# siboehm/NormalizingFlowNetwork

Hardware: AMD Instinct MI355X
Metric: log_prob evals/sec (whole node), 10-flow planar+radial chain, y_dim=1 (higher is better)
Workload: dtype f32; 1 GPU; C2: y_dim=1, (planar,radial)x5 chain, batch 2^24 per GPU; batch_per_gpu=16777216, global_batch=16777216, y_dim=1, param_width=32, trainable_base=True, math=fast, parallelism=dp1, mode=forward

## Files before the change

### normalizingflownetwork_amd/csrc/nfn_bf16.h

```cpp
#pragma once
#include <hip/hip_runtime.h>
#include <stdint.h>

namespace nfn {

typedef float f32x4v __attribute__((ext_vector_type(4)));
typedef unsigned int u32x4v __attribute__((ext_vector_type(4)));
typedef __bf16 bf16x2v __attribute__((ext_vector_type(2)));
typedef __bf16 bf16x8v __attribute__((ext_vector_type(8)));
typedef short s16x4v __attribute__((ext_vector_type(4)));
typedef __attribute__((address_space(3))) s16x4v lds_s16x4v;

__device__ __forceinline__ uint32_t pk_bf16(float a, float b) {
  const bf16x2v v = {(__bf16)a, (__bf16)b};
  return __builtin_bit_cast(uint32_t, v);
}
__device__ __forceinline__ float bf16_lo(uint32_t u) { return __uint_as_float(u << 16); }
__device__ __forceinline__ float bf16_hi(uint32_t u) { return __uint_as_float(u & 0xffff0000u); }
__device__ __forceinline__ void split3_pk(float a, float b, uint32_t& hi, uint32_t& mi, uint32_t& lo) {
  hi = pk_bf16(a, b);
  const float ra = a - bf16_lo(hi), rb = b - bf16_hi(hi);
  mi = pk_bf16(ra, rb);
  lo = pk_bf16(ra - bf16_lo(mi), rb - bf16_hi(mi));
}
__device__ __forceinline__ bf16x8v frag8(uint32_t a, uint32_t b, uint32_t c, uint32_t d) {
  const u32x4v v = {a, b, c, d};
  return __builtin_bit_cast(bf16x8v, v);
}
__device__ __forceinline__ bf16x8v frag8(u32x4v v) { return __builtin_bit_cast(bf16x8v, v); }
__device__ __forceinline__ f32x4v mfma_bf16(bf16x8v a, bf16x8v b, f32x4v c) {
  return __builtin_amdgcn_mfma_f32_16x16x32_bf16(a, b, c, 0, 0, 0);
}

}
```

### normalizingflownetwork_amd/csrc/nfn_dense.hip

```cpp
#include "nfn_bf16.h"
#include "nfn_launch.h"

namespace nfn {
namespace {

typedef float f32x4v __attribute__((ext_vector_type(4)));

template <int DM, bool FAST, int NVH>
__global__ void __launch_bounds__(kMaxBlock) chain_dense_kernel(DenseArgs da) {
  const ChainArgs& a = da.c;
  extern __shared__ float lds[];
  __shared__ double red[2 * kMaxBlock / 64];
  const int tid = threadIdx.x;
  const int lane = tid & 63;
  const int wid = tid >> 6;
  const int H = da.H;
  const int QH = H >> 2;
  const int SH = da.h_lds_stride;
  const int S = a.lds_stride;
  const int P = a.P;
  const int NN = (P + 15) >> 4;
  const int NK = QH;
  const int NP = NN * 16;
  float* wl = lds;
// ... 133 lines not shown
  const int ak = lane >> 4;
  constexpr bool kBReg = QH * NN <= 16;
  float bvr[kBReg ? QH : 1][kBReg ? NN : 1];
  if constexpr (kBReg && !SB) {
#pragma unroll
    for (int ks = 0; ks < QH; ++ks)
#pragma unroll
      for (int nt = 0; nt < NN; ++nt) bvr[ks][nt] = wl[(4 * ks + ak) * NP + 16 * nt + am];
  }
  bf16x8v wsb[SB ? NN : 1][3];
  if constexpr (SB) {
#pragma unroll
    for (int nt = 0; nt < NN; ++nt) {
      uint32_t w1[4], w2[4], w3[4];
#pragma unroll
      for (int q = 0; q < 4; ++q) {
        const int k0 = 8 * (ak & 1) + 2 * q;
        split3_pk(wl[k0 * NP + 16 * nt + am], wl[(k0 + 1) * NP + 16 * nt + am], w1[q], w2[q], w3[q]);
      }
      const bool lo = ak < 2;
      wsb[nt][0] = lo ? frag8(w1[0], w1[1], w1[2], w1[3]) : frag8(w2[0], w2[1], w2[2], w2[3]);
      wsb[nt][1] = lo ? frag8(w3[0], w3[1], w3[2], w3[3]) : frag8(w2[0], w2[1], w2[2], w2[3]);
      wsb[nt][2] = frag8(w1[0], w1[1], w1[2], w1[3]);
    }
  }
  const int64_t hs = da.h_rowstride;
  const int64_t ntiles = a.ntiles;
  const int64_t u0 = (int64_t)blockIdx.x * (blockDim.x >> 6) + wid;
  const int64_t ustep = (int64_t)gridDim.x * (blockDim.x >> 6);
  const bool norm = a.y_mean != nullptr;
  float ymean = 0.0f, ystd = 1.0f, corr = 0.0f;
  if (norm) {
    ymean = a.y_mean[0];
    ystd = a.y_std[0];
    corr = f_log<true>(ystd);
  }
  const int yoff = lane * (int)a.y_bstride * 4;
  const int hoff = (r0 * (int)hs + 4 * c4) * 4;
  const int kstep = RSTEP * (int)hs * 4;
  float4 buf[QH];
  float ybuf;
  auto issue = [&](int64_t tile) {
    if (diag_ablate_loads(a)) tile = u0;
    const int64_t b0 = tile * 64;
    const int64_t nr = max((int64_t)0, min((int64_t)64, a.B - b0));
    const int64_t b0c = nr > 0 ? b0 : 0;
    const auto ry = tile_rsrc(a.y + b0c * a.y_bstride, nr > 0 ? ((nr - 1) * a.y_bstride + 1) * 4 : 0);
    ybuf = __builtin_bit_cast(float, __builtin_amdgcn_raw_buffer_load_b32(ry, yoff, 0, 0));
    const auto rh = tile_rsrc(da.h + b0c * hs, nr > 0 ? ((nr - 1) * hs + H) * 4 : 0);
#pragma unroll
    for (int k = 0; k < QH; ++k)
      buf[k] = __builtin_bit_cast(float4, __builtin_amdgcn_raw_buffer_load_b128(rh, hoff, k * kstep, kNT));
  };
  double acc_sum = 0.0;
  int nfc = 0;
  __amdgpu_buffer_rsrc_t pend_r = tile_rsrc(a.out, 0);
  float pend_v = 0.0f;
  auto flush = [&]() {
    __builtin_amdgcn_raw_buffer_store_b32(__builtin_bit_cast(uint32_t, pend_v), pend_r, lane * 4, 0, kNT);
  };
  issue(u0);
  flush();
  for (int64_t tile = u0; tile < ntiles; tile += ustep) {
    const int64_t b0 = tile * 64;
    const int64_t nr = max((int64_t)0, min((int64_t)64, a.B - b0));
    if constexpr (SB) {
#pragma unroll
      for (int k = 0; k < QH; ++k) {
        uint32_t p1[2], p2[2], p3[2];
        split3_pk(buf[k].x, buf[k].y, p1[0], p2[0], p3[0]);
        split3_pk(buf[k].z, buf[k].w, p1[1], p2[1], p3[1]);
        uint32_t* dst = reinterpret_cast<uint32_t*>(hl) + (r0 + k * RSTEP) * 8 + 2 * c4;
        *reinterpret_cast<uint2*>(dst) = make_uint2(p1[0], p1[1]);
        *reinterpret_cast<uint2*>(dst + kSbPlane) = make_uint2(p2[0], p2[1]);
        *reinterpret_cast<uint2*>(dst + 2 * kSbPlane) = make_uint2(p3[0], p3[1]);
      }
    } else {
#pragma unroll
      for (int k = 0; k < QH; ++k) {
        float* dst = hl + l0 + k * RSTEP * SH;
        dst[0] = buf[k].x;
        dst[1] = buf[k].y;
        dst[2] = buf[k].z;
        dst[3] = buf[k].w;
      }
    }
    const float z0 = norm ? f_div<true>(ybuf - ymean, ystd) : ybuf;
    wave_lds_sync();
    issue(tile + ustep);
    flush();
    if constexpr (SB) {
      const uint32_t* pl = reinterpret_cast<const uint32_t*>(hl) + 4 * (ak & 1);
      const int pa = ak < 2 ? 2 * kSbPlane : kSbPlane, pc = ak < 2 ? kSbPlane : 0;
      f32x4v acc[NN][4];
#pragma unroll
      for (int mt = 0; mt < 4; ++mt) {
        const uint32_t* row = pl + (16 * mt + am) * 8;
        const bf16x8v h0 = frag8(*reinterpret_cast<const u32x4v*>(row + pa));
        const bf16x8v h1 = frag8(*reinterpret_cast<const u32x4v*>(row));
        const bf16x8v h2 = frag8(*reinterpret_cast<const u32x4v*>(row + pc));
#pragma unroll
        for (int nt = 0; nt < NN; ++nt) {
          acc[nt][mt] = mfma_bf16(h0, wsb[nt][0], f32x4v{0.0f, 0.0f, 0.0f, 0.0f});
          acc[nt][mt] = mfma_bf16(h1, wsb[nt][1], acc[nt][mt]);
          acc[nt][mt] = mfma_bf16(h2, wsb[nt][2], acc[nt][mt]);
        }
      }
#pragma unroll
      for (int nt = 0; nt < NN; ++nt) {
        const int n = 16 * nt + am;
        if (n < P) {
          const float bn = da.bias ? da.bias[n] : 0.0f;
#pragma unroll
          for (int mt = 0; mt < 4; ++mt)
            *reinterpret_cast<f32x4v*>(tl + n * kCS + 16 * mt + 4 * ak) = acc[nt][mt] + bn;
        }
      }
    } else {
    float av[4][QH];
#pragma unroll
    for (int mt = 0; mt < 4; ++mt)
#pragma unroll
      for (int ks = 0; ks < QH; ++ks) av[mt][ks] = hl[(16 * mt + am) * SH + 4 * ks + ak];
#pragma unroll
    for (int nt = 0; nt < NN; ++nt) {
      f32x4v acc[4];
#pragma unroll
      for (int mt = 0; mt < 4; ++mt) acc[mt] = f32x4v{0.0f, 0.0f, 0.0f, 0.0f};
#pragma unroll
      for (int ks = 0; ks < QH; ++ks) {
        const float bv = kBReg ? bvr[kBReg ? ks : 0][kBReg ? nt : 0] : wl[(4 * ks + ak) * NP + 16 * nt + am];
#pragma unroll
        for (int mt = 0; mt < 4; ++mt) acc[mt] = __builtin_amdgcn_mfma_f32_16x16x4f32(av[mt][ks], bv, acc[mt], 0, 0, 0);
      }
      const int n = 16 * nt + am;
      if (n < P) {
        const float bn = da.bias ? da.bias[n] : 0.0f;
#pragma unroll
        for (int mt = 0; mt < 4; ++mt)
          *reinterpret_cast<f32x4v*>(tl + n * kCS + 16 * mt + 4 * ak) = acc[mt] + bn;
      }
    }
    }
    wave_lds_sync();
    const float lp = (a.prog.K <= 16 ? eval_chain1_fast<true, kCS, CM, false>(z0, tl + lane, a)
                                     : eval_chain1_fast<false, kCS, kChainLoop, false>(z0, tl + lane, a)) - corr;
    if (lane < nr) {
      acc_sum += (double)lp;
      nfc += nonfinite1(lp);
    }
    pend_v = lp;
    pend_r = tile_rsrc(a.out && nr > 0 ? a.out + b0 : a.out, a.out ? nr * 4 : 0);
    wave_lds_sync();
  }
  flush();
  if (a.partials) {
    write_partial(a.partials, acc_sum, nfc, red, a.out_sum, a.epoch, a.pair_base);
  }
}

template <int QH, int NN, int CM = kChainLoop>
__global__ void __launch_bounds__(kMaxBlock) posterior_dense1_kernel(DenseArgs da) {
  const ChainArgs& a = da.c;
  extern __shared__ float lds[];
  __shared__ double red[2 * kMaxBlock / 64];
  constexpr int RSTEP = 64 / QH;
  constexpr int kNT = 2;
  const int tid = threadIdx.x;
  const int lane = tid & 63;
  const int wid = __builtin_amdgcn_readfirstlane(tid >> 6);
  const int SH = da.h_lds_stride;
  const int P = a.P;
  const int S = a.S;
  float* hl = lds + wid * dense1_wave_floats(P, SH);
  float* tl = hl;
  const int r0 = lane / QH, c4 = lane % QH;
  const int l0 = r0 * SH + 4 * c4;
  const int am = lane & 15, ak = lane >> 4;
  const int64_t hs = da.h_rowstride;
  const int64_t ntiles = a.ntiles;
  const int64_t u0 = (int64_t)blockIdx.x * (blockDim.x >> 6) + wid;
  const int64_t ustep = (int64_t)gridDim.x * (blockDim.x >> 6);
  const bool norm = a.y_mean != nullptr;
  float ymean = 0.0f, ystd = 1.0f, corr = 0.0f;
  if (norm) {
    ymean = a.y_mean[0];
    ystd = a.y_std[0];
    corr = f_log<true>(ystd);
  }
  const int yoff = lane * (int)a.y_bstride * 4;
  const int hoff = (r0 * (int)hs + 4 * c4) * 4;
  const int kstep = RSTEP * (int)hs * 4;
  int woff[QH][NN];
  bool wcol[NN];
#pragma unroll
  for (int nt = 0; nt < NN; ++nt) {
    wcol[nt] = 16 * nt + am < P;
#pragma unroll
    for (int ks = 0; ks < QH; ++ks) woff[ks][nt] = wcol[nt] ? ((4 * ks + ak) * P + 16 * nt + am) * 4 : 0;
  }
  float4 buf[QH];
  float ybuf;
  float wbuf[QH][NN], bbuf[NN];
  auto issue = [&](int64_t tile, int sd) {
    const int64_t b0 = tile * 64;
    const int64_t nr = max((int64_t)0, min((int64_t)64, a.B - b0));
    const int64_t b0c = nr > 0 ? b0 : 0;
    const auto ry = tile_rsrc(a.y + b0c * a.y_bstride, nr > 0 ? ((nr - 1) * a.y_bstride + 1) * 4 : 0);
    ybuf = __builtin_bit_cast(float, __builtin_amdgcn_raw_buffer_load_b32(ry, yoff, 0, 0));
    const auto rh = tile_rsrc(da.h + sd * da.h_drawstride + b0c * hs, nr > 0 ? ((nr - 1) * hs + 4 * QH) * 4 : 0);
#pragma unroll
    for (int k = 0; k < QH; ++k)
      buf[k] = __builtin_bit_cast(float4, __builtin_amdgcn_raw_buffer_load_b128(rh, hoff, k * kstep, kNT));
    const auto rw = tile_rsrc(da.W + sd * da.w_drawstride, nr > 0 ? (int64_t)4 * QH * P * 4 : 0);
#pragma unroll
    for (int ks = 0; ks < QH; ++ks)
#pragma unroll
      for (int nt = 0; nt < NN; ++nt)
        wbuf[ks][nt] = __builtin_bit_cast(float, __builtin_amdgcn_raw_buffer_load_b32(rw, woff[ks][nt], 0, 0));
    const auto rb = tile_rsrc(da.bias ? da.bias + sd * da.b_drawstride : da.W, (da.bias && nr > 0) ? P * 4 : 0);
#pragma unroll
    for (int nt = 0; nt < NN; ++nt)
      bbuf[nt] = __builtin_bit_cast(float, __builtin_amdgcn_raw_buffer_load_b32(rb, (16 * nt + am) * 4, 0, 0));
  };
  double acc_sum = 0.0;
  int nfc = 0;
  __amdgpu_buffer_rsrc_t pend_r = tile_rsrc(a.out, 0);
  float pend_v = 0.0f;
  auto flush = [&]() {
    __builtin_amdgcn_raw_buffer_store_b32(__builtin_bit_cast(uint32_t, pend_v), pend_r, lane * 4, 0, kNT);
  };
  issue(u0, 0);
  flush();
  for (int64_t tile = u0; tile < ntiles; tile += ustep) {
    const int64_t b0 = tile * 64;
    const int64_t nr = max((int64_t)0, min((int64_t)64, a.B - b0));
    float m = -INFINITY, lacc = 0.0f;
    for (int sd = 0; sd < S; ++sd) {
#pragma unroll
      for (int k = 0; k < QH; ++k) {
        float* dst = hl + l0 + k * RSTEP * SH;
        dst[0] = buf[k].x;
        dst[1] = buf[k].y;
        dst[2] = buf[k].z;
        dst[3] = buf[k].w;
      }
      float wv[QH][NN], bv[NN];
#pragma unroll
      for (int nt = 0; nt < NN; ++nt) {
        bv[nt] = bbuf[nt];
#pragma unroll
        for (int ks = 0; ks < QH; ++ks) wv[ks][nt] = wcol[nt] ? wbuf[ks][nt] : 0.0f;
      }
      const float z0 = norm ? f_div<true>(ybuf - ymean, ystd) : ybuf;
      wave_lds_sync();
      const bool last = sd + 1 == S;
      issue(last ? tile + ustep : tile, last ? 0 : sd + 1);
      flush();
      pend_r = tile_rsrc(a.out, 0);
      float av[4][QH];
#pragma unroll
      for (int mt = 0; mt < 4; ++mt)
#pragma unroll
        for (int ks = 0; ks < QH; ++ks) av[mt][ks] = hl[(16 * mt + am) * SH + 4 * ks + ak];
#pragma unroll
      for (int nt = 0; nt < NN; ++nt) {
        f32x4v acc[4];
#pragma unroll
        for (int mt = 0; mt < 4; ++mt) acc[mt] = f32x4v{0.0f, 0.0f, 0.0f, 0.0f};
#pragma unroll
        for (int ks = 0; ks < QH; ++ks)
#pragma unroll
          for (int mt = 0; mt < 4; ++mt) acc[mt] = __builtin_amdgcn_mfma_f32_16x16x4f32(av[mt][ks], wv[ks][nt], acc[mt], 0, 0, 0);
        const int n = 16 * nt + am;
        if (n < P) {
#pragma unroll
          for (int mt = 0; mt < 4; ++mt)
            *reinterpret_cast<f32x4v*>(tl + n * kCS + 16 * mt + 4 * ak) = acc[mt] + bv[nt];
        }
      }
      wave_lds_sync();
      const float lp = (a.prog.K <= 16 ? eval_chain1_fast<true, kCS, CM, false>(z0, tl + lane, a)
                                       : eval_chain1_fast<false, kCS, kChainLoop, false>(z0, tl + lane, a)) - corr;
      lse_push<true>(m, lacc, lp);
      wave_lds_sync();
    }
    const float res = lse_finish<true>(m, lacc, S);
    if (lane < nr) {
      acc_sum += (double)res;
      nfc += nonfinite1(res);
    }
    pend_v = res;
    pend_r = tile_rsrc(a.out && nr > 0 ? a.out + b0 : a.out, a.out ? nr * 4 : 0);
  }
  flush();
  if (a.partials) {
    write_partial(a.partials, acc_sum, nfc, red, a.out_sum, a.epoch, a.pair_base);
  }
}

template <int DM, bool FAST>
__global__ void __launch_bounds__(kMaxBlock) posterior_dense_kernel(DenseArgs da) {
  const ChainArgs& a = da.c;
  extern __shared__ float lds[];
  __shared__ double red[2 * kMaxBlock / 64];
  const int tid = threadIdx.x;
// ... 203 lines not shown
        for (int ks = 0; ks < QH; ++ks) av[mt][ks] = hl[(16 * mt + am) * SH + 4 * ks + ak];
#pragma unroll
      for (int nt = 0; nt < NNMAX; ++nt) {
        if (nt < NN) {
          f32x4v acc[4];
#pragma unroll
          for (int mt = 0; mt < 4; ++mt) acc[mt] = f32x4v{0.0f, 0.0f, 0.0f, 0.0f};
#pragma unroll
          for (int ks = 0; ks < QH; ++ks)
#pragma unroll
            for (int mt = 0; mt < 4; ++mt)
              acc[mt] = __builtin_amdgcn_mfma_f32_16x16x4f32(av[mt][ks], wv[ks][nt], acc[mt], 0, 0, 0);
          const int n = 16 * nt + am;
          if (n < P) {
#pragma unroll
            for (int mt = 0; mt < 4; ++mt) {
#pragma unroll
              for (int i = 0; i < 4; ++i) tl[(16 * mt + 4 * ak + i) * S + n] = acc[mt][i] + bv[nt];
            }
          }
        }
      }
      wave_lds_sync();
      float z[DM];
#pragma unroll
      for (int j = 0; j < DM; ++j) z[j] = z0[j];
      const float lp = eval_chain<DM, true>(z, tl + lane * S, a) - corr;
      lse_push<true>(m, lacc, lp);
      wave_lds_sync();
    }
    const float res = lse_finish<true>(m, lacc, ND);
    if (lane < nr) {
      acc_sum += (double)res;
      nfc += nonfinite1(res);
    }
    pend_v = res;
    pend_r = tile_rsrc(a.out && nr > 0 ? a.out + b0 : a.out, a.out ? nr * 4 : 0);
  }
  flush();
  if (a.partials) {
    write_partial(a.partials, acc_sum, nfc, red, a.out_sum, a.epoch, a.pair_base);
  }
}

template <int DM, int QH>
void launch_pdp(const DenseArgs& da, hipStream_t s, int64_t* grid_out) {
  auto kfn = posterior_densep_kernel<DM, QH>;
  const size_t lds = (size_t)(4 * (64 * da.h_lds_stride + 64 * da.c.lds_stride) + 16) * sizeof(float);
  const int64_t grid = persistent_grid(kfn, kMaxBlock, lds, (da.c.ntiles + 3) / 4);
  *grid_out = std::max<int64_t>(1, grid);
  nfn_launch(kfn, dim3((unsigned)*grid_out), dim3(kMaxBlock), lds, s, da);
}

template <int DM>
bool launch_pdp_h(const DenseArgs& da, hipStream_t s, int64_t* g) {
  switch (da.H >> 2) {
    case 1: launch_pdp<DM, 1>(da, s, g); return true;
    case 2: launch_pdp<DM, 2>(da, s, g); return true;
    case 4: launch_pdp<DM, 4>(da, s, g); return true;
  }
  return false;
}

template <int QH, int CM>
void launch_pd1_form(const DenseArgs& da, hipStream_t s, int64_t* grid_out) {
  const int nn = (da.c.P + 15) >> 4;
  const size_t lds = (size_t)(4 * dense1_wave_floats(da.c.P, da.h_lds_stride) + 16) * sizeof(float);
  auto kfn = nn <= 1 ? posterior_dense1_kernel<QH, 1, CM>
                     : (nn == 2 ? posterior_dense1_kernel<QH, 2, CM> : (nn == 3 ? posterior_dense1_kernel<QH, 3, CM>
                                                                                : posterior_dense1_kernel<QH, 4, CM>));
  int64_t grid = persistent_grid(kfn, kMaxBlock, lds, (da.c.ntiles + 3) / 4);
  *grid_out = std::max<int64_t>(1, grid);
  nfn_launch(kfn, dim3((unsigned)*grid_out), dim3(kMaxBlock), lds, s, da);
}

#ifndef NFN_DENSE_HP
template <int QH>
void launch_pd1(const DenseArgs& da, hipStream_t s, int64_t* grid_out) {
  int cm = env_int("NFN_CHAIN_FORM", -1);
  if (cm < 0 && hpair_types(da.c) >= 0) cm = kChainHPair;
  if (cm == kChainHPair && launch_dense1_hpair(hpair_types(da.c), true, da, s, grid_out)) return;
  if (cm == kChainLoop)
    launch_pd1_form<QH, kChainLoop>(da, s, grid_out);
  else
    launch_pd1_form<QH, kChainPairs>(da, s, grid_out);
}

template <int DM, bool FAST>
void launch_pd(const DenseArgs& da, hipStream_t s, int64_t* grid_out) {
  auto kfn = posterior_dense_kernel<DM, FAST>;
  const size_t lds = (size_t)(4 * (64 * da.h_lds_stride + 64 * da.c.lds_stride) + 16) * sizeof(float);
  const int64_t grid = persistent_grid(kfn, kMaxBlock, lds, (da.c.ntiles + 3) / 4);
  *grid_out = std::max<int64_t>(1, grid);
  nfn_launch(kfn, dim3((unsigned)*grid_out), dim3(kMaxBlock), lds, s, da);
}

template <bool FAST>
bool launch_pd_dm(int dm, const DenseArgs& da, hipStream_t s, int64_t* g) {
  const ChainArgs& a = da.c;
  if constexpr (FAST) {
    if (dm == 1 && a.d == 1 && env_int("NFN_DENSE1", 1) != 0 && da.h_rowstride * 256 < ((int64_t)1 << 31) &&
        a.y_bstride * 256 < ((int64_t)1 << 31)) {
      switch (da.H >> 2) {
        case 1: launch_pd1<1>(da, s, g); return true;
        case 2: launch_pd1<2>(da, s, g); return true;
        case 4: launch_pd1<4>(da, s, g); return true;
        case 8: launch_pd1<8>(da, s, g); return true;
      }
    }
  }
  if constexpr (FAST) {
    if (dm >= 2 && a.d >= 2 && da.H <= 16 && env_int("NFN_DENSEP", 1) != 0 && da.h_rowstride * 256 < ((int64_t)1 << 31) &&
        a.y_bstride * 256 < ((int64_t)1 << 31)) {
      bool ok = false;
      switch (dm) {
        case 2: ok = launch_pdp_h<2>(da, s, g); break;
        case 4: ok = launch_pdp_h<4>(da, s, g); break;
        case 8: ok = launch_pdp_h<8>(da, s, g); break;
      }
      if (ok) return true;
    }
  }
  switch (dm) {
    case 1: launch_pd<1, FAST>(da, s, g); return true;
    case 2: launch_pd<2, FAST>(da, s, g); return true;
    case 4: launch_pd<4, FAST>(da, s, g); return true;
    case 8: launch_pd<8, FAST>(da, s, g); return true;
  }
  return false;
}

#endif

constexpr int kDenseSplitBf16 = 1;
template <int QH, int CM>
void launch_d1_form(const DenseArgs& da, hipStream_t s, int64_t* grid_out) {
  const int nn = (da.c.P + 15) >> 4;
  bool sb = false;
  if constexpr (QH == 4) sb = nn <= 2 && env_int("NFN_DENSE_SB", kDenseSplitBf16) != 0;
  const int wf = sb ? dense1_sb_wave_floats(da.c.P, da.h_lds_stride) : dense1_wave_floats(da.c.P, da.h_lds_stride);
  const size_t lds = (size_t)(4 * QH * nn * 16 + 4 * wf + 16) * sizeof(float);
  auto kfn = nn <= 1 ? chain_dense1_kernel<QH, 1, CM>
                     : (nn == 2 ? chain_dense1_kernel<QH, 2, CM> : (nn == 3 ? chain_dense1_kernel<QH, 3, CM>
                                                                           : chain_dense1_kernel<QH, 4, CM>));
  if constexpr (QH == 4) {
    if (sb) kfn = nn <= 1 ? chain_dense1_kernel<QH, 1, CM, true> : chain_dense1_kernel<QH, 2, CM, true>;
  }
  int64_t grid = persistent_grid(kfn, kMaxBlock, lds, (da.c.ntiles + 3) / 4);
  *grid_out = std::max<int64_t>(1, grid);
  nfn_launch(kfn, dim3((unsigned)*grid_out), dim3(kMaxBlock), lds, s, da);
}

#ifndef NFN_DENSE_HP
template <int QH>
void launch_d1(const DenseArgs& da, size_t , hipStream_t s, int64_t* grid_out) {
  int cm = env_int("NFN_CHAIN_FORM", -1);
  if (cm < 0 && hpair_types(da.c) >= 0) cm = kChainHPair;
  if (cm == kChainHPair && launch_dense1_hpair(hpair_types(da.c), false, da, s, grid_out)) return;
#ifdef NFN_DIAG
  if (cm == kStaticProg && (da.c.P + 15) >> 4 == 2 && da.c.prog.K == kStaticK[0] &&
      da.c.prog.types[0] == kStaticTypes[0]) {
    launch_d1_form<QH, kStaticProg>(da, s, grid_out);
    return;
  }
  if (cm == kChainLoop) {
    launch_d1_form<QH, kChainLoop>(da, s, grid_out);
    return;
  }
#endif
  launch_d1_form<QH, kChainPairs>(da, s, grid_out);
}
#endif

#ifndef NFN_DENSE_HP
template <int DM, bool FAST, int NVH>
void launch_d(const DenseArgs& da, size_t lds, hipStream_t s, int64_t* grid_out) {
  auto kfn = chain_dense_kernel<DM, FAST, NVH>;
  const int64_t grid = persistent_grid(kfn, kMaxBlock, lds, (da.c.ntiles + 3) / 4);
  *grid_out = std::max<int64_t>(1, grid);
  nfn_launch(kfn, dim3((unsigned)*grid_out), dim3(kMaxBlock), lds, s, da);
}

template <int DM, bool FAST>
bool launch_d_h(int nvh, const DenseArgs& da, size_t lds, hipStream_t s, int64_t* g) {
  switch (nvh) {
    case 1: launch_d<DM, FAST, 1>(da, lds, s, g); return true;
    case 2: launch_d<DM, FAST, 2>(da, lds, s, g); return true;
    case 4: launch_d<DM, FAST, 4>(da, lds, s, g); return true;
    case 8: launch_d<DM, FAST, 8>(da, lds, s, g); return true;
    case 16: launch_d<DM, FAST, 16>(da, lds, s, g); return true;
  }
  return false;
}

template <bool FAST>
bool launch_d_dm(int dm, int nvh, const DenseArgs& da, size_t lds, hipStream_t s, int64_t* g) {
  const ChainArgs& a = da.c;
  if constexpr (FAST) {
    if (dm == 1 && a.d == 1 && env_int("NFN_DENSE1", 1) != 0 && da.h_rowstride * 256 < ((int64_t)1 << 31) &&
        a.y_bstride * 256 < ((int64_t)1 << 31)) {
      switch (nvh) {
        case 1: launch_d1<1>(da, lds, s, g); return true;
        case 2: launch_d1<2>(da, lds, s, g); return true;
        case 4: launch_d1<4>(da, lds, s, g); return true;
        case 8: launch_d1<8>(da, lds, s, g); return true;
      }
    }
  }
  switch (dm) {
    case 1: return launch_d_h<1, FAST>(nvh, da, lds, s, g);
    case 2: return launch_d_h<2, FAST>(nvh, da, lds, s, g);
    case 4: return launch_d_h<4, FAST>(nvh, da, lds, s, g);
    case 8: return launch_d_h<8, FAST>(nvh, da, lds, s, g);
  }
  return false;
}

#endif

}

#ifdef NFN_DENSE_HP
#define NFN_CAT2(a, b) a##b
#define NFN_CAT(a, b) NFN_CAT2(a, b)
#define NFN_DENSE_HP_FN NFN_CAT(launch_dense1_hpair_, NFN_DENSE_HP)
bool NFN_DENSE_HP_FN(bool post, const DenseArgs& da, hipStream_t s, int64_t* g) {
  constexpr int CM = hpair_form(NFN_DENSE_HP / 3, NFN_DENSE_HP % 3, 1);
  switch (da.H >> 2) {
    case 1: post ? launch_pd1_form<1, CM>(da, s, g) : launch_d1_form<1, CM>(da, s, g); return true;
    case 2: post ? launch_pd1_form<2, CM>(da, s, g) : launch_d1_form<2, CM>(da, s, g); return true;
    case 4: post ? launch_pd1_form<4, CM>(da, s, g) : launch_d1_form<4, CM>(da, s, g); return true;
    case 8: post ? launch_pd1_form<8, CM>(da, s, g) : launch_d1_form<8, CM>(da, s, g); return true;
  }
  return false;
}
#else
bool launch_dense1_hpair(int sel, bool post, const DenseArgs& da, hipStream_t s, int64_t* grid) {
  switch (sel) {
    case 0: return launch_dense1_hpair_0(post, da, s, grid);
    case 1: return launch_dense1_hpair_1(post, da, s, grid);
    case 3: return launch_dense1_hpair_3(post, da, s, grid);
    case 4: return launch_dense1_hpair_4(post, da, s, grid);
  }
  return false;
}

bool launch_dense(bool fast, int dm, int nvh, const DenseArgs& da, size_t lds, hipStream_t s, int64_t* grid) {
  return fast ? launch_d_dm<true>(dm, nvh, da, lds, s, grid) : launch_d_dm<false>(dm, nvh, da, lds, s, grid);
}

bool launch_posterior_dense(bool fast, int dm, const DenseArgs& da, hipStream_t s, int64_t* grid) {
  return fast ? launch_pd_dm<true>(dm, da, s, grid) : launch_pd_dm<false>(dm, da, s, grid);
}
#endif

}
```

### normalizingflownetwork_amd/csrc/nfn_device.h

```cpp
#pragma once

#include <hip/hip_runtime.h>

#include <math.h>
#include <stdint.h>
#include <stdlib.h>
#include <string.h>

#include <algorithm>

#include "nfn.h"

#pragma clang fp contract(on)

#if defined(__HIP_DEVICE_COMPILE__) && !defined(__gfx950__)
#error "the nfn kernels are written for gfx950 (MI355X) only"
#endif

namespace nfn {

constexpr int kMaxBlock = 256;
constexpr int kLdsTileBudget = 48 * 1024;
constexpr int kLdsMaxBytes = 156 * 1024;
constexpr float kSoftplusThr = 13.942384719848633f;
// ... 486 lines not shown
}

#define NFN_PAIR_SWITCH(sel, CALL) \
  switch (sel) {                   \
    case 0: CALL(0, 0); break;     \
    case 1: CALL(0, 1); break;     \
    case 2: CALL(0, 2); break;     \
    case 3: CALL(1, 0); break;     \
    case 4: CALL(1, 1); break;     \
    case 5: CALL(1, 2); break;     \
    case 6: CALL(2, 0); break;     \
    case 7: CALL(2, 1); break;     \
    default: CALL(2, 2); break;    \
  }

__device__ __forceinline__ int type1(uint32_t types, int k) { return (int)((types >> ((2 * k) & 31)) & 3u); }

template <int ST = 1, bool ACCM = true>
__device__ __forceinline__ float chain1_fast_pairs(float& z, const float* row, uint32_t types, int K, int P) {
  float l2 = 0.0f;
  int ia = type1(types, 0), ib = type1(types, 1);
  int offa = max(P - size1(ia), 0), offb = max(offa - size1(ib), 0);
  float pa[3], pb[3];
  read3c<ST>(pa, row, offa);
  read3c<ST>(pb, row, offb);
#pragma unroll 1
  for (int k = 0; k + 1 < K; k += 2) {
    const int ian = type1(types, k + 2), ibn = type1(types, k + 3);
    const int offan = max(offb - size1(ian), 0), offbn = max(offan - size1(ibn), 0);
    float pna[3], pnb[3];
    read3c<ST>(pna, row, offan);
    read3c<ST>(pnb, row, offbn);
#define NFN_FWD(A, B) flow_pair1<A, B, ACCM>(z, l2, pa, pb)
    NFN_PAIR_SWITCH(ia * 3 + ib, NFN_FWD)
#undef NFN_FWD
    ia = ian;
    ib = ibn;
    offb = offbn;
#pragma unroll
    for (int i = 0; i < 3; ++i) {
      pa[i] = pna[i];
      pb[i] = pnb[i];
    }
  }
  if (K & 1) l2 += __builtin_amdgcn_logf(fabsf(flow1_fast<ACCM>(ia, z, pa)));
  return l2;
}

template <int IA, int IB, int U, int ST = 1, bool ACCM = true>
__device__ __forceinline__ float chain1_fast_hpairs(float& z, const float* row, int K, int P) {
  constexpr int SA = IA == NFN_FLOW_AFFINE ? 2 : 3, SB = IB == NFN_FLOW_AFFINE ? 2 : 3, SP = SA + SB;
  float l2 = 0.0f;
  int off = P;
  const int np = K >> 1;
  int p = 0;
  if constexpr (U == 0) {
    float pa[3], pb[3];
    read3c<ST>(pa, row, max(off - SA, 0));
    read3c<ST>(pb, row, max(off - SP, 0));
#pragma unroll 1
    for (; p < np; ++p) {
      off -= SP;
      float pna[3], pnb[3];
      read3c<ST>(pna, row, max(off - SA, 0));
      read3c<ST>(pnb, row, max(off - SP, 0));
      flow_pair1<IA, IB, ACCM>(z, l2, pa, pb);
#pragma unroll
      for (int i = 0; i < 3; ++i) {
        pa[i] = pna[i];
        pb[i] = pnb[i];
      }
    }
    if (K & 1) l2 += __builtin_amdgcn_logf(fabsf(flow1_fast<ACCM>(IA, z, pa)));
    return l2;
  }
#pragma unroll 1
  for (; p + U <= np; p += U) {
    float pa[U > 0 ? U : 1][3], pb[U > 0 ? U : 1][3];
#pragma unroll
    for (int u = 0; u < U; ++u) {
      read3c<ST>(pa[u], row, off - u * SP - SA);
      read3c<ST>(pb[u], row, off - u * SP - SP);
    }
#pragma unroll
    for (int u = 0; u < U; ++u) flow_pair1<IA, IB, ACCM>(z, l2, pa[u], pb[u]);
    off -= U * SP;
  }
#pragma unroll 1
  for (; p < np; ++p) {
    float pa[3], pb[3];
    read3c<ST>(pa, row, off - SA);
    read3c<ST>(pb, row, off - SP);
    flow_pair1<IA, IB, ACCM>(z, l2, pa, pb);
    off -= SP;
  }
  if (K & 1) {
    float pa[3];
    read3c<ST>(pa, row, off - SA);
    l2 += __builtin_amdgcn_logf(fabsf(flow1_fast<ACCM>(IA, z, pa)));
  }
  return l2;
}

template <int ST = 1>
__device__ __forceinline__ void chain1_fast_pairs2(float& za, float& zb, const float* rowa, const float* rowb,
                                                   uint32_t types, int K, int P, float& l2a, float& l2b) {
  l2a = 0.0f;
  l2b = 0.0f;
  int ia = type1(types, 0), ib = type1(types, 1);
  int offa = max(P - size1(ia), 0), offb = max(offa - size1(ib), 0);
  float pa[3], pb[3], qa[3], qb[3];
  read3c<ST>(pa, rowa, offa);
  read3c<ST>(pb, rowa, offb);
  read3c<ST>(qa, rowb, offa);
  read3c<ST>(qb, rowb, offb);
#pragma unroll 1
  for (int k = 0; k + 1 < K; k += 2) {
    const int ian = type1(types, k + 2), ibn = type1(types, k + 3);
    const int offan = max(offb - size1(ian), 0), offbn = max(offan - size1(ibn), 0);
    float pna[3], pnb[3], qna[3], qnb[3];
    read3c<ST>(pna, rowa, offan);
    read3c<ST>(pnb, rowa, offbn);
    read3c<ST>(qna, rowb, offan);
    read3c<ST>(qnb, rowb, offbn);
#define NFN_FWD2(A, B)                   \
  flow_pair1<A, B>(za, l2a, pa, pb);     \
  flow_pair1<A, B>(zb, l2b, qa, qb)
    NFN_PAIR_SWITCH(ia * 3 + ib, NFN_FWD2)
#undef NFN_FWD2
    ia = ian;
    ib = ibn;
    offb = offbn;
#pragma unroll
    for (int i = 0; i < 3; ++i) {
      pa[i] = pna[i];
      pb[i] = pnb[i];
      qa[i] = qna[i];
      qb[i] = qnb[i];
    }
  }
  if (K & 1) {
    l2a += __builtin_amdgcn_logf(fabsf(flow1_fast(ia, za, pa)));
    l2b += __builtin_amdgcn_logf(fabsf(flow1_fast(ia, zb, qa)));
  }
}

constexpr int kChainLoop = 0, kStaticProg = 2, kChainPairs = 3, kStaticCache = 4, kStaticCacheX = 5;
constexpr int kChainHPair = 8;
constexpr int hpair_form(int ia, int ib, int u) { return kChainHPair + 9 * u + 3 * ia + ib; }
constexpr int kPairsMaxKStream = 4;
constexpr uint32_t kStaticTypes[] = {0x44444u};
constexpr int kStaticK[] = {10};

template <int ST = 1>
__device__ __forceinline__ float base1_fast(float z, const float* row, bool trainable) {
  if (trainable) {
    const float sc = 1e-3f + sp_fast1(kLogExpm1One + 0.1f * row[ST]);
    const float zz = f_div<true>(z - row[0], sc);
    return -0.5f * (zz * zz) - (kHalfLog2Pi + __builtin_amdgcn_logf(sc) * kLn2);
  }
  return -0.5f * (z * z) - kHalfLog2Pi;
}

template <bool PACKED, int ST = 1, int CM = kChainLoop, bool ACCM = true>
__device__ __forceinline__ float eval_chain1_fast(float z, const float* row, const ChainArgs& a) {
  const int K = a.prog.K;
  float l2 = 0.0f;
  if constexpr (CM >= kChainHPair) {
    constexpr int c = CM - kChainHPair;
    l2 = chain1_fast_hpairs<(c % 9) / 3, c % 3, c / 9, ST, ACCM>(z, row, K, a.P);
  } else if constexpr (CM == kChainPairs) {
    if (K > 0) l2 = chain1_fast_pairs<ST, ACCM>(z, row, a.prog.types[0], K, a.P);
  } else if constexpr (CM == kStaticProg) {
    l2 = chain1_fast_static<kStaticTypes[0], kStaticK[0], ST, ACCM>(z, row, a.P);
  } else if constexpr (PACKED) {
    if (K > 0) l2 = chain1_fast_packed<ST, ACCM>(z, row, a.prog.types[0], K, a.P);
  } else if (K > 0) {
    int st = a.prog.step[0];
    float pc[3];
    read3<ST>(pc, row, st);
    for (int k = 0; k < K; ++k) {
      const int stn = (k + 1 < K) ? a.prog.step[k + 1] : 0;
      float pn[3];
      if (k + 1 < K) read3<ST>(pn, row, stn);
      const int id = st & 3;
      float l;
      if (id == NFN_FLOW_PLANAR)
        l = planar1_fast<ACCM>(z, pc[0], pc[1], pc[2]);
      else if (id == NFN_FLOW_RADIAL)
        l = radial1_fast(z, pc[0], pc[1], pc[2]);
      else
        l = affine1_fast(z, pc[0], pc[1]);
      l2 += __builtin_amdgcn_logf(fabsf(l));
      st = stn;
      pc[0] = pn[0];
      pc[1] = pn[1];
      pc[2] = pn[2];
    }
  }
  return base1_fast<ST>(z, row, a.trainable != 0) + l2 * kLn2;
}

template <int DM, bool FAST>
__device__ __forceinline__ float eval_sample(float (&z)[DM], const float* row, const ChainArgs& a) {
  if constexpr (DM == 1 && FAST)
    return eval_chain1_fast<false>(z[0], row, a);
  else
    return eval_chain<DM, FAST>(z, row, a);
}

__device__ __forceinline__ void stage_rows(float* lds, const float* __restrict__ src, int64_t rs, int nr,
                                           int P, int S, bool vec4) {
  const int nth = blockDim.x;
  const int tid = threadIdx.x;
  if (vec4) {
    const int q = P >> 2;
    const int n = nr * q;
    const int step_r = nth / q, step_c = nth - (nth / q) * q;
    int r = tid / q, c = tid - (tid / q) * q;
    for (int i = tid; i < n; i += nth) {
      const float4 v = *reinterpret_cast<const float4*>(src + (int64_t)r * rs + 4 * c);
      float* dst = lds + r * S + 4 * c;
      dst[0] = v.x;
      dst[1] = v.y;
      dst[2] = v.z;
      dst[3] = v.w;
      r += step_r;
      c += step_c;
      if (c >= q) {
        c -= q;
        r += 1;
      }
    }
  } else {
    const int n = nr * P;
    const int step_r = nth / P, step_c = nth - (nth / P) * P;
    int r = tid / P, c = tid - (tid / P) * P;
    for (int i = tid; i < n; i += nth) {
      lds[r * S + c] = src[(int64_t)r * rs + c];
      r += step_r;
      c += step_c;
      if (c >= P) {
        c -= P;
        r += 1;
      }
    }
  }
}

__device__ __forceinline__ double block_sum(double v, double* red) {
#pragma unroll
  for (int off = 32; off > 0; off >>= 1) v += __shfl_xor(v, off);
  const int wid = threadIdx.x >> 6;
  if ((threadIdx.x & 63) == 0) red[wid] = v;
  __syncthreads();
  double s = 0.0;
  if (threadIdx.x == 0) {
    const int nw = (blockDim.x + 63) >> 6;
    for (int w = 0; w < nw; ++w) s += red[w];
  }
  return s;
}

__device__ __forceinline__ int nonfinite1(float v) { return __builtin_isfinite(v) ? 0 : 1; }

constexpr int kSumWaves = 4;
template <bool ATOMIC = false>
__device__ __forceinline__ void sum_pairs(const double* __restrict__ pairs, int64_t n, double* red, double* out) {
  const int lane = threadIdx.x & 63, nw = (int)(blockDim.x >> 6), wid = (int)(threadIdx.x >> 6);
  for (int k = wid; k < kSumWaves; k += nw) {
    double s = 0.0, c = 0.0;
    for (int64_t i = 64 * k + lane; i < n; i += 64 * kSumWaves) {
      if constexpr (ATOMIC) {
        s += __hip_atomic_load(pairs + 2 * i, __ATOMIC_RELAXED, __HIP_MEMORY_SCOPE_AGENT);
        c += __hip_atomic_load(pairs + 2 * i + 1, __ATOMIC_RELAXED, __HIP_MEMORY_SCOPE_AGENT);
      } else {
        s += pairs[2 * i];
        c += pairs[2 * i + 1];
      }
    }
#pragma unroll
    for (int off = 32; off > 0; off >>= 1) {
      s += __shfl_xor(s, off);
      c += __shfl_xor(c, off);
    }
    if (lane == 0) {
      red[2 * k] = s;
      red[2 * k + 1] = c;
    }
  }
  __syncthreads();
  if (threadIdx.x == 0) {
    double ts = 0.0, tc = 0.0;
    for (int k = 0; k < kSumWaves; ++k) {
      ts += red[2 * k];
      tc += red[2 * k + 1];
    }
    out[0] = ts;
    out[1] = tc;
  }
}

__device__ __forceinline__ void write_partial(double* partials, double acc, int nf, double* red,
                                              double* out_sum, uint32_t epoch, int64_t base = 0) {
  double c = (double)nf;
#pragma unroll
  for (int off = 32; off > 0; off >>= 1) {
    acc += __shfl_xor(acc, off);
    c += __shfl_xor(c, off);
  }
  const int wid = threadIdx.x >> 6;
  if ((threadIdx.x & 63) == 0) {
    red[2 * wid] = acc;
    red[2 * wid + 1] = c;
// ... 1060 lines not shown
```

Baseline: 43.91 billion evals/s.

## Add register-resident dense1 kernel using 32x32 MFMA for fixed 10-flow chains

Adds a specialized kernel for H=16, P=32 and 10-flow planar/radial or radial-only chains with a trainable base. Each wave computes its 64-row tile's parameter projection with 32x32x16 bf16 MFMAs on a three-way bf16 split, loading h straight into registers, and swaps halves with permlane32. The flow chain is then evaluated entirely from registers with a compile-time unrolled type sequence. This is meant to remove the LDS staging and generic chain loop of the existing kernel, at the cost of more registers and a narrow specialization.

Result: no change. 43.86 billion evals/s (-0.1%).

```diff
diff --git a/normalizingflownetwork_amd/csrc/nfn_bf16.h b/normalizingflownetwork_amd/csrc/nfn_bf16.h
--- a/normalizingflownetwork_amd/csrc/nfn_bf16.h
+++ b/normalizingflownetwork_amd/csrc/nfn_bf16.h
@@ -31,5 +31,9 @@
 __device__ __forceinline__ f32x4v mfma_bf16(bf16x8v a, bf16x8v b, f32x4v c) {
   return __builtin_amdgcn_mfma_f32_16x16x32_bf16(a, b, c, 0, 0, 0);
 }
+typedef float f32x16v __attribute__((ext_vector_type(16)));
+__device__ __forceinline__ f32x16v mfma32_bf16(bf16x8v a, bf16x8v b, f32x16v c) {
+  return __builtin_amdgcn_mfma_f32_32x32x16_bf16(a, b, c, 0, 0, 0);
+}
 
 }
diff --git a/normalizingflownetwork_amd/csrc/nfn_dense.hip b/normalizingflownetwork_amd/csrc/nfn_dense.hip
--- a/normalizingflownetwork_amd/csrc/nfn_dense.hip
+++ b/normalizingflownetwork_amd/csrc/nfn_dense.hip
@@ -309,6 +309,153 @@
     pend_v = lp;
     pend_r = tile_rsrc(a.out && nr > 0 ? a.out + b0 : a.out, a.out ? nr * 4 : 0);
     wave_lds_sync();
+  }
+  flush();
+  if (a.partials) {
+    write_partial(a.partials, acc_sum, nfc, red, a.out_sum, a.epoch, a.pair_base);
+  }
+}
+
+template <uint32_t TYPES, int K, int HM, int BI, bool PB>
+__global__ void __launch_bounds__(kMaxBlock) chain_dense1_reg_kernel(DenseArgs da) {
+  constexpr int H = 16, P = 32;
+  static_assert(P == 2 + 3 * K, "planar / radial flows and a trainable base");
+  const ChainArgs& a = da.c;
+  extern __shared__ float lds[];
+  __shared__ double red[2 * kMaxBlock / 64];
+  constexpr int kAux = HM == 1 ? 0 : 2;
+  const int tid = threadIdx.x;
+  const int lane = tid & 63;
+  const int wid = __builtin_amdgcn_readfirstlane(tid >> 6);
+  const int ln = lane & 31, hg = lane >> 5;
+  uint32_t* hl = reinterpret_cast<uint32_t*>(lds) + wid * 3 * kSbPlane;
+  bf16x8v w1, w2, w3;
+  {
+    uint32_t p1[4], p2[4], p3[4];
+#pragma unroll
+    for (int q = 0; q < 4; ++q) {
+      const int k0 = 8 * hg + 2 * q;
+      split3_pk(da.W[k0 * P + ln], da.W[(k0 + 1) * P + ln], p1[q], p2[q], p3[q]);
+    }
+    w1 = frag8(p1[0], p1[1], p1[2], p1[3]);
+    w2 = frag8(p2[0], p2[1], p2[2], p2[3]);
+    w3 = frag8(p3[0], p3[1], p3[2], p3[3]);
+  }
+  f32x16v bi;
+#pragma unroll
+  for (int r = 0; r < 16; ++r) bi[r] = BI == 1 && da.bias ? da.bias[8 * (r >> 2) + 4 * hg + (r & 3)] : 0.0f;
+  float bs[BI == 0 ? P : 1];
+  if constexpr (BI == 0) {
+#pragma unroll
+    for (int p = 0; p < P; ++p) bs[p] = da.bias ? da.bias[p] : 0.0f;
+  }
+  const int64_t hs = da.h_rowstride;
+  const int64_t ntiles = a.ntiles;
+  const int64_t u0 = (int64_t)blockIdx.x * (blockDim.x >> 6) + wid;
+  const int64_t ustep = (int64_t)gridDim.x * (blockDim.x >> 6);
+  const bool norm = a.y_mean != nullptr;
+  float ymean = 0.0f, ystd = 1.0f, corr = 0.0f;
+  if (norm) {
+    ymean = a.y_mean[0];
+    ystd = a.y_std[0];
+    corr = f_log<true>(ystd);
+  }
+  const int yoff = lane * (int)a.y_bstride * 4;
+  const int r0 = lane >> 2, c4 = lane & 3;
+  const int hoff = HM == 0 ? (r0 * (int)hs + 4 * c4) * 4 : (ln * (int)hs + 8 * hg) * 4;
+  const int kstep = (HM == 0 ? 16 : 32) * (int)hs * 4;
+  float4 buf[4];
+  float ybuf;
+  auto issue = [&](int64_t tile) {
+    if (diag_ablate_loads(a)) tile = u0;
+    const int64_t b0 = tile * 64;
+    const int64_t nr = max((int64_t)0, min((int64_t)64, a.B - b0));
+    const int64_t b0c = nr > 0 ? b0 : 0;
+    const auto ry = tile_rsrc(a.y + b0c * a.y_bstride, nr > 0 ? ((nr - 1) * a.y_bstride + 1) * 4 : 0);
+    ybuf = __builtin_bit_cast(float, __builtin_amdgcn_raw_buffer_load_b32(ry, yoff, 0, 0));
+    const auto rh = tile_rsrc(da.h + b0c * hs, nr > 0 ? ((nr - 1) * hs + H) * 4 : 0);
+#pragma unroll
+    for (int k = 0; k < 4; ++k) {
+      const int off = HM == 0 ? hoff + k * kstep : hoff + (k >> 1) * kstep + 16 * (k & 1);
+      buf[k] = __builtin_bit_cast(float4, __builtin_amdgcn_raw_buffer_load_b128(rh, off, 0, kAux));
+    }
+  };
+  double acc_sum = 0.0;
+  int nfc = 0;
+  __amdgpu_buffer_rsrc_t pend_r = tile_rsrc(a.out, 0);
+  float pend_v = 0.0f;
+  auto flush = [&]() {
+    __builtin_amdgcn_raw_buffer_store_b32(__builtin_bit_cast(uint32_t, pend_v), pend_r, lane * 4, 0, 2);
+  };
+  issue(u0);
+  flush();
+  for (int64_t tile = u0; tile < ntiles; tile += ustep) {
+    const int64_t b0 = tile * 64;
+    const int64_t nr = max((int64_t)0, min((int64_t)64, a.B - b0));
+    bf16x8v hb[2][3];
+    if constexpr (HM == 0) {
+#pragma unroll
+      for (int k = 0; k < 4; ++k) {
+        uint32_t p1[2], p2[2], p3[2];
+        split3_pk(buf[k].x, buf[k].y, p1[0], p2[0], p3[0]);
+        split3_pk(buf[k].z, buf[k].w, p1[1], p2[1], p3[1]);
+        uint32_t* dst = hl + (r0 + 16 * k) * 8 + 2 * c4;
+        *reinterpret_cast<uint2*>(dst) = make_uint2(p1[0], p1[1]);
+        *reinterpret_cast<uint2*>(dst + kSbPlane) = make_uint2(p2[0], p2[1]);
+        *reinterpret_cast<uint2*>(dst + 2 * kSbPlane) = make_uint2(p3[0], p3[1]);
+      }
+    } else {
+#pragma unroll
+      for (int hf = 0; hf < 2; ++hf) {
+        uint32_t p1[4], p2[4], p3[4];
+#pragma unroll
+        for (int k = 0; k < 2; ++k) {
+          const float4 v = buf[2 * hf + k];
+          split3_pk(v.x, v.y, p1[2 * k], p2[2 * k], p3[2 * k]);
+          split3_pk(v.z, v.w, p1[2 * k + 1], p2[2 * k + 1], p3[2 * k + 1]);
+        }
+        hb[hf][0] = frag8(p1[0], p1[1], p1[2], p1[3]);
+        hb[hf][1] = frag8(p2[0], p2[1], p2[2], p2[3]);
+        hb[hf][2] = frag8(p3[0], p3[1], p3[2], p3[3]);
+      }
+    }
+    const float z0 = norm ? f_div<true>(ybuf - ymean, ystd) : ybuf;
+    if constexpr (HM == 0) wave_lds_sync();
+    issue(tile + ustep);
+    flush();
+    if constexpr (HM == 0) {
+#pragma unroll
+      for (int hf = 0; hf < 2; ++hf)
+#pragma unroll
+        for (int p = 0; p < 3; ++p)
+          hb[hf][p] = frag8(*reinterpret_cast<const u32x4v*>(hl + p * kSbPlane + (32 * hf + ln) * 8 + 4 * hg));
+      wave_lds_sync();
+    }
+    f32x16v X = mfma32_bf16(w1, hb[0][2], bi), Y = mfma32_bf16(w1, hb[1][2], bi);
+    X = mfma32_bf16(w3, hb[0][0], X), Y = mfma32_bf16(w3, hb[1][0], Y);
+    X = mfma32_bf16(w2, hb[0][1], X), Y = mfma32_bf16(w2, hb[1][1], Y);
+    X = mfma32_bf16(w1, hb[0][1], X), Y = mfma32_bf16(w1, hb[1][1], Y);
+    X = mfma32_bf16(w2, hb[0][0], X), Y = mfma32_bf16(w2, hb[1][0], Y);
+    X = mfma32_bf16(w1, hb[0][0], X), Y = mfma32_bf16(w1, hb[1][0], Y);
+    float t[P];
+#pragma unroll
+    for (int r = 0; r < 16; ++r) {
+      const auto sw = __builtin_amdgcn_permlane32_swap(__builtin_bit_cast(uint32_t, (float)X[r]),
+                                                       __builtin_bit_cast(uint32_t, (float)Y[r]), false, false);
+      t[8 * (r >> 2) + (r & 3)] = __builtin_bit_cast(float, (uint32_t)sw[0]);
+      t[8 * (r >> 2) + 4 + (r & 3)] = __builtin_bit_cast(float, (uint32_t)sw[1]);
+    }
+    if constexpr (BI == 0) {
+#pragma unroll
+      for (int p = 0; p < P; ++p) t[p] += bs[p];
+    }
+    const float lp = eval_chain1_fast_reg<TYPES, K, P, false, PB>(z0, t) - corr;
+    if (lane < nr) {
+      acc_sum += (double)lp;
+      nfc += nonfinite1(lp);
+    }
+    pend_v = lp;
+    pend_r = tile_rsrc(a.out && nr > 0 ? a.out + b0 : a.out, a.out ? nr * 4 : 0);
   }
   flush();
   if (a.partials) {
@@ -818,9 +965,56 @@
 }
 
 #ifndef NFN_DENSE_HP
+constexpr int kDenseReg = 3, kDenseRegBias = 1, kDenseRegPB = 0;
+constexpr uint32_t kRegTypesPR5 = 0x44444u, kRegTypesR10 = 0x55555u;
+template <uint32_t TYPES, int HM, int BI, bool PB>
+void launch_d1_reg_form(const DenseArgs& da, hipStream_t s, int64_t* grid_out) {
+  auto kfn = chain_dense1_reg_kernel<TYPES, 10, HM, BI, PB>;
+  const size_t lds = HM == 0 ? (size_t)(4 * 3 * kSbPlane) * sizeof(float) : 0;
+  const int64_t grid = persistent_grid(kfn, kMaxBlock, lds, (da.c.ntiles + 3) / 4);
+  *grid_out = std::max<int64_t>(1, grid);
+  nfn_launch(kfn, dim3((unsigned)*grid_out), dim3(kMaxBlock), lds, s, da);
+}
+template <uint32_t TYPES>
+void launch_d1_reg(int hm, const DenseArgs& da, hipStream_t s, int64_t* grid_out) {
+#ifdef NFN_DIAG
+  const int bi = env_int("NFN_DENSE_REG_BIAS", kDenseRegBias) != 0, pb = env_int("NFN_DENSE_REG_PB", kDenseRegPB) != 0;
+  switch (4 * (hm - 1) + 2 * bi + pb) {
+    case 0: return launch_d1_reg_form<TYPES, 0, 0, false>(da, s, grid_out);
+    case 1: return launch_d1_reg_form<TYPES, 0, 0, true>(da, s, grid_out);
+    case 2: return launch_d1_reg_form<TYPES, 0, 1, false>(da, s, grid_out);
+    case 3: return launch_d1_reg_form<TYPES, 0, 1, true>(da, s, grid_out);
+    case 4: return launch_d1_reg_form<TYPES, 1, 0, false>(da, s, grid_out);
+    case 5: return launch_d1_reg_form<TYPES, 1, 0, true>(da, s, grid_out);
+    case 6: return launch_d1_reg_form<TYPES, 1, 1, false>(da, s, grid_out);
+    case 7: return launch_d1_reg_form<TYPES, 1, 1, true>(da, s, grid_out);
+    case 8: return launch_d1_reg_form<TYPES, 2, 0, false>(da, s, grid_out);
+    case 9: return launch_d1_reg_form<TYPES, 2, 0, true>(da, s, grid_out);
+    case 10: return launch_d1_reg_form<TYPES, 2, 1, false>(da, s, grid_out);
+    default: return launch_d1_reg_form<TYPES, 2, 1, true>(da, s, grid_out);
+  }
+#else
+  static_assert(kDenseReg == 3 && kDenseRegBias == 1 && kDenseRegPB == 0, "the release form");
+  launch_d1_reg_form<TYPES, 2, 1, false>(da, s, grid_out);
+#endif
+}
+inline bool launch_d1_reg_program(const DenseArgs& da, hipStream_t s, int64_t* grid_out) {
+  const int hm = env_int("NFN_DENSE_REG", kDenseReg);
+  const ChainArgs& a = da.c;
+  if (hm < 1 || hm > 3 || da.H != 16 || a.P != 32 || a.trainable == 0 || a.prog.K != 10) return false;
+  if (a.prog.types[0] == kRegTypesPR5)
+    launch_d1_reg<kRegTypesPR5>(hm, da, s, grid_out);
+  else if (a.prog.types[0] == kRegTypesR10)
+    launch_d1_reg<kRegTypesR10>(hm, da, s, grid_out);
+  else
+    return false;
+  return true;
+}
+
 template <int QH>
 void launch_d1(const DenseArgs& da, size_t , hipStream_t s, int64_t* grid_out) {
   int cm = env_int("NFN_CHAIN_FORM", -1);
+  if (cm < 0 && launch_d1_reg_program(da, s, grid_out)) return;
   if (cm < 0 && hpair_types(da.c) >= 0) cm = kChainHPair;
   if (cm == kChainHPair && launch_dense1_hpair(hpair_types(da.c), false, da, s, grid_out)) return;
 #ifdef NFN_DIAG
diff --git a/normalizingflownetwork_amd/csrc/nfn_device.h b/normalizingflownetwork_amd/csrc/nfn_device.h
--- a/normalizingflownetwork_amd/csrc/nfn_device.h
+++ b/normalizingflownetwork_amd/csrc/nfn_device.h
@@ -662,14 +662,30 @@
 constexpr uint32_t kStaticTypes[] = {0x44444u};
 constexpr int kStaticK[] = {10};
 
+__device__ __forceinline__ float base1_fast_trained(float z, float loc, float scraw) {
+  const float sc = 1e-3f + sp_fast1(kLogExpm1One + 0.1f * scraw);
+  const float zz = f_div<true>(z - loc, sc);
+  return -0.5f * (zz * zz) - (kHalfLog2Pi + __builtin_amdgcn_logf(sc) * kLn2);
+}
 template <int ST = 1>
 __device__ __forceinline__ float base1_fast(float z, const float* row, bool trainable) {
-  if (trainable) {
-    const float sc = 1e-3f + sp_fast1(kLogExpm1One + 0.1f * row[ST]);
-    const float zz = f_div<true>(z - row[0], sc);
-    return -0.5f * (zz * zz) - (kHalfLog2Pi + __builtin_amdgcn_logf(sc) * kLn2);
-  }
+  if (trainable) return base1_fast_trained(z, row[0], row[ST]);
   return -0.5f * (z * z) - kHalfLog2Pi;
+}
+
+template <uint32_t TYPES, int K, int P, bool ACCM = true, bool PB = false>
+__device__ __forceinline__ float eval_chain1_fast_reg(float z, const float (&t)[P]) {
+  float l2 = 0.0f;
+  int off = P;
+#pragma unroll
+  for (int k = 0; k < K; ++k) {
+    const int id = (int)((TYPES >> (2 * k)) & 3u);
+    off -= size1(id);
+    const float pc[3] = {t[off], t[off + 1], t[id == NFN_FLOW_AFFINE ? off : off + 2]};
+    l2 += __builtin_amdgcn_logf(fabsf(flow1_fast<ACCM>(id, z, pc)));
+    if (PB && (k & 1)) __builtin_amdgcn_sched_barrier(0);
+  }
+  return base1_fast_trained(z, t[0], t[1]) + l2 * kLn2;
 }
 
 template <bool PACKED, int ST = 1, int CM = kChainLoop, bool ACCM = true>
```
